# dart-icra/DART-Dual-Arm-Non-Prehensile-Manipulation

Hardware: AMD Instinct MI355X
Metric: MPC solves/sec (horizon N=20, batch=18 objects) at 1/2/4/8 GPUs; max |u−u_ref| (higher is better)
Workload: dtype f64

## Files before the change

dart-dual-arm-non-prehensile-manipulation_amd/csrc/dart_mpc_abi.hip:

```cpp
#include "abi_internal.h"

hipError_t device_stage(DeviceStage** out) {
    static DeviceStage stages[64];
    int dev = 0;
    hipError_t e = hipGetDevice(&dev);
    if (e != hipSuccess) return e;
    if (dev < 0 || dev >= 64) return hipErrorInvalidDevice;
    DeviceStage& d = stages[dev];
    std::lock_guard<std::mutex> g(d.mu);
    if (!d.stream) e = hipStreamCreateWithFlags(&d.stream, hipStreamNonBlocking);
    *out = &d;
    return e;
}

namespace {

int check_cfg(const dart_mpc_config* c) {
    if (!c) return 0;
    if (c->variant != DART_MPC_PMPC && c->variant != DART_MPC_RMPC && c->variant != DART_MPC_LMPC) return 0;
    if (c->N < 1 || c->N > 63) return 0;
    if (!(c->Ts > 0.0) || !(c->tol > 0.0) || !(c->gravity == c->gravity) || c->max_iter < 1 || c->B_max < 1) return 0;
    if (c->acceptable_iter < 0 || (c->acceptable_iter > 0 && !(c->acceptable_tol > 0.0))) return 0;
    if (c->max_soc < 0 || c->max_soc > 8) return 0;
    if (c->pmpc_path != 0 && c->pmpc_path != 1) return 0;
    if (!(c->constr_mult_init_max >= 0.0)) return 0;
    if (!(c->max_cpu_time >= 0.0) || c->max_cpu_time > 1e9) return 0;
    return 1;
}

void server_release(dart_mpc_handle* h) {
    auto& v = h->srv;
    if (v.mbox) (void)hipHostFree(v.mbox);
    if (v.stream) (void)hipStreamDestroy(v.stream);
    v = dart_mpc_handle::Server{};
}

void io_release(dart_mpc_handle* h) {
    auto& o = h->io;
    if (o.hin) (void)hipHostFree(o.hin);
    if (o.hout) (void)hipHostFree(o.hout);
    o = dart_mpc_handle::Io{};
}

hipError_t ensure_io(dart_mpc_handle* h) {
// ... 863 lines not shown
```

dart-dual-arm-non-prehensile-manipulation_amd/csrc/pmpc_ipm.hip:

```cpp
#if DART_WG == 2
#define dartmpc dartmpc_wg2
#endif
#include <hip/hip_runtime.h>
#include <stdint.h>
#include <stdlib.h>

#include "pmpc_ipm.h"
#include "pmpc_model.h"
#include "pmpc_resto.h"
#include "stamps.h"
#include "wave.h"

namespace dartmpc {

#ifdef DART_STAMPS
#ifndef PMPC_SEQ
__device__ unsigned long long g_stamp[16];
#define STAMP_FLUSH(b) STAMP_FLUSH_TO(g_stamp, b)
#else
__device__ unsigned long long g_stamp_seq[16];
#define STAMP_FLUSH(b) STAMP_FLUSH_TO(g_stamp_seq, b)
#endif
#else
#define STAMP_FLUSH(b) STAMP_FLUSH_TO(g_stamp, b)
#endif

#if DART_WG == 2
__shared__ double g_pm_x[4][2][4];
#endif
template <int SITE, int NV>
__device__ __forceinline__ void pm_pass(int src_wave, int src_node, const double (&v)[NV], double (&o)[NV]) {
    static_assert(NV <= 4 && SITE < 4, "four slots, four sites");
#if DART_WG == 1
    (void)src_wave; (void)src_node;
#pragma unroll
    for (int i = 0; i < NV; ++i) o[i] = v[i];
#else
    const int l = lane_id();
    if (wave_idx() == src_wave && (l & 31) == src_node) {
#pragma unroll
        for (int i = 0; i < NV; ++i) g_pm_x[SITE][l >> 5][i] = v[i];
    }
    __syncthreads();
#pragma unroll
// ... 55 lines not shown
    double F[16];
#pragma unroll
    for (int e = 0; e < 16; ++e)
        F[e] = fz[e] ? (e == 0 ? 1.0 : 0.0)
                     : (e % 5 == 0) ? dpp_fill<CTRL, 0xf, 1>(T[e]) : dpp_fill<CTRL, 0xf, 0>(T[e]);
    double N[16];
#pragma unroll
    for (int i = 0; i < 4; ++i)
#pragma unroll
        for (int j = 0; j < 4; ++j) {
            double acc = T[4 * i + 3] * F[12 + j];
            if (fz[12 + j]) acc = 0.0;
            acc = fma(T[4 * i + 2], F[8 + j], acc);
            if (!fz[4 + j]) acc = fma(T[4 * i + 1], F[4 + j], acc);
            if (FIRST && i == 0) acc += F[j];
            else if (!(FIRST && (i == 1 || i == 3))) acc = fma(T[4 * i], F[j], acc);
            N[4 * i + j] = acc;
        }
#pragma unroll
    for (int e = 0; e < 16; ++e) T[e] = N[e];
}

#define PM_EXPECT(x, v) (ONEROW ? (bool)(x) : (bool)__builtin_expect((long)(bool)(x), (v)))

struct PmStage {
    double f11, a12k, a22k, ai12k, ai22k, a22i, uonf, A11k, A12k, A22k;
};

template <int NAX, bool QSCAN, bool ONEROW, bool SHORT2>
__device__ __forceinline__ bool pmpc_riccati(const int lane, const int N, const bool uon, const bool lsm,
                                             const double delta, const double qp2, const double qv2,
                                             const PmStage& c, const double (&be1)[NAX], const double (&be2)[NAX],
                                             const double (&E11)[NAX], const double (&E12)[NAX],
                                             const double (&E22)[NAX], const double (&Rt0)[NAX], double (&P11)[NAX],
                                             double (&P12)[NAX], double (&P22)[NAX], double (&W1)[NAX],
                                             double (&W2)[NAX], double (&iQs)[NAX], bool& use_scan) {
    constexpr bool one_row = ONEROW;
    constexpr bool short2 = SHORT2 && !ONEROW;
    const double f11 = c.f11, a12k = c.a12k, a22k = c.a22k, ai12k = c.ai12k, ai22k = c.ai22k, a22i = c.a22i;
    const double uonf = c.uonf, A11k = c.A11k, A12k = c.A12k, A22k = c.A22k;
    (void)lane; (void)ai12k; (void)ai22k; (void)a22i; (void)uonf;
    const double X11d = lsm ? 1.0 : qp2 + delta, X22d = lsm ? 1.0 : qv2 + delta;
    double Quu[NAX], Rt[NAX];
#pragma unroll
    for (int j = 0; j < NAX; ++j) {
        P11[j] = X11d; P12[j] = 0.0; P22[j] = X22d;
// ... 122 lines not shown
        for (int j = 0; j < NAX; ++j) {
            const double e1 = be1[j], e2 = be2[j];
            const double Q = fma(E11[j], n11[j], fma(E12[j], n12[j], fma(E22[j], n22[j], Rt[j])));
            const double PB1 = fma(n11[j], e1, n12[j] * e2), PB2 = fma(n12[j], e1, n22[j] * e2);
            const double U1 = PB1, U2 = fma(PB1, a12k, PB2 * a22k);
            const double X12 = fma(n11[j], a12k, n12[j] * a22k);
            const double X22 = fma(A11k, n11[j], fma(A12k, n12[j], fma(A22k, n22[j], X22d)));
            const double iQ = frcp(Q);
            const double w1 = iQ * U1, w2 = iQ * U2;
            P11[j] = fma(-w1, U1, fma(f11, n11[j], X11d));
            P12[j] = fma(-w1, U2, X12);
            P22[j] = fma(-w2, U2, X22);
            W1[j] = w1; W2[j] = w2;
            Quu[j] = Q; iQs[j] = iQ;
        }
    }
    bool bad = false;
#pragma unroll
    for (int j = 0; j < NAX; ++j) bad = bad || !(Quu[j] > 0.0) || !isfinite(Quu[j]);
    return !wany(bad);
}

struct PmOvlShared {
    double pt[6][kWave];
    double fc[6][kWave];
    int flag[4];
};
__shared__ PmOvlShared g_pm_ovl;

template <int NAX, bool QSCAN, bool ONEROW, bool SHORT2, bool RED, bool OVL = false>
__device__ __forceinline__ bool pmpc_solve(const PmpcArgs& a, const int b) {
    static_assert(!OVL || (NAX == 1 && QSCAN && !ONEROW && !RED && kWaves == 1), "the overlapped build: scan builds of N = 16..31");
    STAMP_DECL
    const int lane = (kWaves == 1 && !OVL) ? (int)threadIdx.x : lane_id();
    const int k = NAX == 1 ? node_base() + (lane & 31) : lane;
    const int ax0 = NAX == 1 ? (lane >> 5) : 0;
    const int N = a.N;
    const bool xon = k <= N, uon = k < N;
    constexpr bool one_row = ONEROW;
    constexpr bool short2 = SHORT2 && !ONEROW;
    const double h = a.Ts;

    const double* st = a.x0 + 6 * b;
    const double* rf = a.ref + 6 * b;
    const double* pr = a.prm + 6 * b;
    const double mu_f = pr[0], Qp = pr[1], Qv = pr[2], R = pr[3], ulo = pr[4], uhi = pr[5];

    double a12, a22, b1, b2;
    axis_rk4(h, a.g, mu_f, 0.0, 0.0, 1.0, a12, a22);
// ... 26 lines not shown
        v[j] = xon ? (ww ? ww[6 * k + 2 * ax + 1] : sv[j]) : 0.0;
        double t = uon ? (ww ? ww[6 * (N + 1) + 2 * k + ax] : 0.0) : 0.0;
        if (uon) t = fmin(fmax(t, lo + pushl), hi - pushu);
        th[j] = t;
        lp[j] = 0.0; lv[j] = 0.0;
        zl[j] = uon ? 1.0 : 0.0; zu[j] = uon ? 1.0 : 0.0;
        if (xon) gmax = fmax(gmax, fmax(fabs(2 * Qp * (p[j] - rp[j])), fabs(2 * Qv * (v[j] - rv[j]))));
        if (uon) gmax = fmax(gmax, fabs(2 * R * th[j]));
        zA[j] = ax ? zav : zp1; zC[j] = ax ? zcv : zcp;
        zs[j] = st[4 + ax];
        zz[j] = xon ? (ww ? ww[6 * k + 4 + ax] : zs[j]) : 0.0;
    }
    gmax = wmax(gmax);
    const double sc = gmax > 100.0 ? 100.0 / gmax : 1.0;
    const double qp2 = sc * 2 * Qp, qv2 = sc * 2 * Qv, r2 = sc * 2 * R;
    const double scQp = sc * Qp, scQv = sc * Qv, scR = sc * R;
    const PmStage stg = {f11, a12k, a22k, ai12k, ai22k, a22i, uonf, A11k, A12k, A22k};
    auto quad_stage = [&](double csj, double snj, double lpnj, double lvnj, double zlj, double islj, double zuj,
                          double isuj, double& e1, double& e2, double& e11, double& e12, double& e22, double& rt0) {
        e1 = b1 * csj; e2 = b2 * csj;
        e11 = e1 * e1; e12 = 2.0 * e1 * e2; e22 = e2 * e2;
        rt0 = uon ? fma(snj, fma(b1, lpnj, b2 * lvnj), r2 + zlj * islj + zuj * isuj) : 1.0;
    };
    if constexpr (OVL) {
        if (__builtin_amdgcn_readfirstlane((int)(threadIdx.x >> 6)) != 0) {
            const long long max_rounds = 2ll * a.max_iter + 8;
            for (long long round = 0; round < max_rounds; ++round) {
                __syncthreads();
                if (__builtin_amdgcn_readfirstlane(g_pm_ovl.flag[0])) return false;
#ifdef DART_STAMPS
                const unsigned long long tf0 = __builtin_amdgcn_s_memtime();
#endif
                const double th1 = g_pm_ovl.pt[0][lane], sn1 = g_pm_ovl.pt[1][lane];
                const double lp1 = g_pm_ovl.pt[2][lane], lv1 = g_pm_ovl.pt[3][lane];
                const double zl1 = g_pm_ovl.pt[4][lane], zu1 = g_pm_ovl.pt[5][lane];
                const double c_ = tilt_cos_econ(poly, th1);
                const double cs1 = uon ? c_ : 0.0;
                const double ln = from_next(lp1), vn = from_next(lv1);
                const double lpn1 = uon ? ln : 0.0, lvn1 = uon ? vn : 0.0;
                const double sl = th1 - lo, su = hi - th1;
                const double isl1 = uon ? frcp(sl) : 0.0, isu1 = uon ? frcp(su) : 0.0;
                double be1[NAX], be2[NAX], E11[NAX], E12[NAX], E22[NAX], Rt0[NAX];
                quad_stage(cs1, sn1, lpn1, lvn1, zl1, isl1, zu1, isu1, be1[0], be2[0], E11[0], E12[0], E22[0], Rt0[0]);
                double W1[NAX], W2[NAX], P11[NAX], P12[NAX], P22[NAX], iQs[NAX];
                bool us = false;
                const bool okf = pmpc_riccati<NAX, QSCAN, ONEROW, SHORT2>(lane, N, uon, false, 0.0, qp2, qv2, stg, be1,
                                                                         be2, E11, E12, E22, Rt0, P11, P12, P22, W1,
                                                                         W2, iQs, us);
                g_pm_ovl.fc[0][lane] = P11[0]; g_pm_ovl.fc[1][lane] = P12[0]; g_pm_ovl.fc[2][lane] = P22[0];
                g_pm_ovl.fc[3][lane] = W1[0]; g_pm_ovl.fc[4][lane] = W2[0]; g_pm_ovl.fc[5][lane] = iQs[0];
                if (lane == 0) { g_pm_ovl.flag[1] = us ? 1 : 0; g_pm_ovl.flag[2] = okf ? 1 : 0; }
#ifdef DART_STAMPS
                t_acc_[13] += __builtin_amdgcn_s_memtime() - tf0;
                if (lane == 0) g_pm_ovl.flag[3] = (int)t_acc_[13];
#endif
                __syncthreads();
                if (__builtin_amdgcn_readfirstlane(g_pm_ovl.flag[0])) return false;
            }
            return false;
        }
        if (lane == 0) g_pm_ovl.flag[0] = 0;
    }

    const double tol = a.tol, mu_min = tol / 10;
    const double n_eq = 6.0 * (N + 1), n_b = 4.0 * N;
    const double inv_neb = 1.0 / (n_eq + n_b), inv_nb = 1.0 / n_b;
    const double gam_th = 1e-5, gam_ph = 1e-8, s_th = 1.1, s_ph = 2.3, eta_ph = 1e-8, gam_al = 0.05;

    auto defects = [&](double pj, double vj, double sj, double spj, double svj, double& g1, double& g2) {
        const double fp = fma(a12, vj, fma(b1, sj, pj));
        const double fv = fma(a22, vj, b2 * sj);
        double ip, iv;
        if constexpr (kWaves == 1) {
            ip = from_prev(fp); iv = from_prev(fv);
        } else {
            const double x2[2] = {fp, fv};
            double o2[2];
            from_prev_n(x2, o2);
            ip = o2[0]; iv = o2[1];
        }
        g1 = (k == 0) ? pj - spj : pj - ip;
        g2 = (k == 0) ? vj - svj : vj - iv;
    };
    auto axes_sum = [&](const double (&q)[NAX]) -> double {
        if constexpr (NAX == 1) return half_pair_sum(q[0]);
        else return q[0] + q[1];
    };
    auto zdefect = [&](double zj, double wj, int j) -> double {
        const double fz = fma(zA[j], zj, zC[j] * wj);
        const double ip = from_prev(fz);
        return (k == 0) ? zj - zs[j] : zj - ip;
    };
    auto vz_new = [&](const double (&t)[NAX]) -> double {
        double sq[NAX];
#pragma unroll
        for (int j = 0; j < NAX; ++j) sq[j] = uon ? t[j] * t[j] : 0.0;
        return -a.g * axes_sum(sq);
    };

    double g1[NAX], g2[NAX], gz[NAX], snc[NAX];
    double lgc[NAX];
    (void)lgc;
    double th0 = 0.0;
    {
        const double w0 = vz_new(th);
#pragma unroll
        for (int j = 0; j < NAX; ++j) {
            double s0, c0_;
            tilt_sincos(poly, th[j], s0, c0_);
            snc[j] = uon ? s0 : 0.0;
            if constexpr (OVL) lgc[j] = log_fast((th[j] - lo) * (hi - th[j]));
            defects(p[j], v[j], snc[j], sp[j], sv[j], g1[j], g2[j]);
            gz[j] = RED ? 0.0 : zdefect(zz[j], w0, j);
            if (xon) th0 += fabs(g1[j]) + fabs(g2[j]) + fabs(gz[j]);
        }
    }
    double theta = wsum(th0);
    const double th_max = 1e4 * fmax(1.0, theta), th_min = 1e-4 * fmax(1.0, theta);

    double fth = 0.0, fph = 0.0;
    int nfilt = 0;
    double mu = 0.1, delta_last = 0.0;
    int status = -1, it = 0;
    int in_soft = 0, soft_count = 0;
    STAMP(0);

    double zsm[4] = {0.0, 0.0, 0.0, 0.0};
    (void)zsm;
    if constexpr (OVL) {
        double m = k == 0 ? 0.0 : zA[0], c = 0.0;
        affine1_scan_level<0x111, 0xf>(m, c); zsm[0] = m;
        affine1_scan_level<0x112, 0xf>(m, c); zsm[1] = m;
        affine1_scan_level<0x114, 0xf>(m, c); zsm[2] = m;
        if constexpr (!short2) { affine1_scan_level<0x118, 0xf>(m, c); zsm[3] = m; }
    }

    bool published = false;
    auto publish = [&]() {
        __builtin_amdgcn_sched_barrier(0);
        g_pm_ovl.pt[0][lane] = th[0]; g_pm_ovl.pt[1][lane] = snc[0];
        g_pm_ovl.pt[2][lane] = lp[0]; g_pm_ovl.pt[3][lane] = lv[0];
        g_pm_ovl.pt[4][lane] = zl[0]; g_pm_ovl.pt[5][lane] = zu[0];
        __syncthreads();
        __builtin_amdgcn_sched_barrier(0);
        published = true;
    };
#ifdef DART_STAMPS
    const unsigned long long t_loop0 = __builtin_amdgcn_s_memtime();
#endif
    for (it = a.mult_init_max > 0.0 ? -1 : 0; it < a.max_iter; ++it) {
        const bool lsm = it < 0;
#ifdef DART_STAMPS
        if (it == 1) t_acc_[12] = __builtin_amdgcn_s_memtime() - t_loop0;
#endif
        if constexpr (OVL) {
            if (PM_EXPECT(!lsm && !published, 0)) publish();
        }
        double sn[NAX], cs[NAX], isl[NAX], isu[NAX], lpn[NAX], lvn[NAX];
        double dinf = 0.0, pinf = 0.0, c0 = 0.0, cmin = 1e300, suml = 0.0, sumz = 0.0;
#pragma unroll
        for (int j = 0; j < NAX; ++j) {
            sn[j] = snc[j];
            const double c_ = tilt_cos_econ(poly, th[j]);
            cs[j] = uon ? c_ : 0.0;
            double ln, vn;
            if constexpr (kWaves == 1) {
                ln = from_next(lp[j]); vn = from_next(lv[j]);
            } else {
                const double x2[2] = {lp[j], lv[j]};
                double o2[2];
                from_next_n(x2, o2);
                ln = o2[0]; vn = o2[1];
            }
            lpn[j] = uon ? ln : 0.0; lvn[j] = uon ? vn : 0.0;
            const double sl = th[j] - lo, su = hi - th[j];
            isl[j] = uon ? frcp(sl) : 0.0; isu[j] = uon ? frcp(su) : 0.0;
            const double r1 = fma(qp2, p[j] - rp[j], lp[j] - lpn[j]);
            const double r2x = fma(qv2, v[j] - rv[j], lv[j] - fma(a12, lpn[j], a22 * lvn[j]));
            const double ru = fma(r2, th[j], -cs[j] * fma(b1, lpn[j], b2 * lvn[j])) - zl[j] + zu[j];
            dinf = fmax(dinf, xon ? fmax(fabs(r1), fabs(r2x)) : 0.0);
            dinf = fmax(dinf, uon ? fabs(ru) : 0.0);
            pinf = fmax(pinf, xon ? fmax(fmax(fabs(g1[j]), fabs(g2[j])), fabs(gz[j])) : 0.0);
            suml += xon ? fabs(lp[j]) + fabs(lv[j]) : 0.0;
            c0 = fmax(c0, uon ? fmax(zl[j] * sl, zu[j] * su) : 0.0);
            cmin = fmin(cmin, uon ? fmin(zl[j] * sl, zu[j] * su) : 1e300);
            sumz += zl[j] + zu[j];
        }
        float dinf_f = (float)dinf, pinf_f = (float)pinf, c0_f = (float)c0, cmin_f = (float)cmin;
        float suml_f = (float)suml, sumz_f = (float)sumz;
        wred_errors(dinf_f, pinf_f, c0_f, cmin_f, suml_f, sumz_f);
        const double dinf_w = dinf_f, pinf_w = pinf_f, c0_w = c0_f;
        const double cmin_w = cmin_f;
        const float sz_w = sumz_f;
        const double is_d = 100.0 * frcp(fmax(100.0, (double)(suml_f + sz_w) * inv_neb));
        const double is_c = 100.0 * frcp(fmax(100.0, (double)sz_w * inv_nb));
        dinf = dinf_w; pinf = pinf_w; c0 = c0_w;
        STAMP(1);
        if (!lsm && fmax(dinf * is_d, fmax(pinf, c0 * is_c)) <= tol) { status = 0; break; }
        for (; !lsm;) {
            const double cmu = fmax(c0 - mu, mu - cmin_w);
            if (fmax(dinf * is_d, fmax(pinf, cmu * is_c)) > 10.0 * mu || mu <= mu_min) break;
            mu = fmax(mu_min, fmin(0.2 * mu, mu * sqrt(mu)));
            nfilt = 0; in_soft = 0;
        }
        const double tau = fmax(0.99, 1.0 - mu);
        STAMP(2);

        double be1[NAX], be2[NAX], E11[NAX], E12[NAX], E22[NAX], Rt0[NAX], rt[NAX], q1[NAX], q2[NAX];
#pragma unroll
        for (int j = 0; j < NAX; ++j) {
            quad_stage(cs[j], sn[j], lpn[j], lvn[j], zl[j], isl[j], zu[j], isu[j], be1[j], be2[j], E11[j], E12[j],
                       E22[j], Rt0[j]);
            rt[j] = uon ? (lsm ? r2 * th[j] - zl[j] + zu[j] : fma(r2, th[j], mu * (isu[j] - isl[j]))) : 0.0;
            q1[j] = qp2 * (p[j] - rp[j]); q2[j] = qv2 * (v[j] - rv[j]);
        }
        double W1[NAX], W2[NAX], P11[NAX], P12[NAX], P22[NAX], iQs[NAX];
        double delta = 0.0;
        bool ok = false;
        int attempt = 0;
        if constexpr (OVL) {
            if (!lsm) {
                __builtin_amdgcn_sched_barrier(0);
                SPAN_BEGIN(t_b);
                __syncthreads();
                SPAN_END(14, t_b);
                const int usf = g_pm_ovl.flag[1], okff = g_pm_ovl.flag[2];
                P11[0] = g_pm_ovl.fc[0][lane]; P12[0] = g_pm_ovl.fc[1][lane]; P22[0] = g_pm_ovl.fc[2][lane];
                W1[0] = g_pm_ovl.fc[3][lane]; W2[0] = g_pm_ovl.fc[4][lane]; iQs[0] = g_pm_ovl.fc[5][lane];
                const bool us = __builtin_amdgcn_readfirstlane(usf) != 0;
                const bool okf = __builtin_amdgcn_readfirstlane(okff) != 0;
                if (PM_EXPECT(us && okf, 1)) {
                    STAMP_ADD(11, 1);
                    ok = true; attempt = 1;
                }
            }
        }
        for (; attempt < 60 && !ok; ++attempt) {
            if (PM_EXPECT(attempt > 0, 0))
                delta = (attempt == 1) ? (delta_last == 0.0 ? 1e-4 : fmax(1e-20, delta_last * (1.0 / 3.0)))
                                       : delta * (delta_last == 0.0 ? 100.0 : 8.0);
            bool use_scan = false;
            ok = pmpc_riccati<NAX, QSCAN, ONEROW, SHORT2>(lane, N, uon, lsm, delta, qp2, qv2, stg, be1, be2, E11, E12,
                                                          E22, Rt0, P11, P12, P22, W1, W2, iQs, use_scan);
            STAMP_ADD(11, use_scan ? 1 : 0);
        }
        STAMP_ADD(9, attempt);
        STAMP(3);
        if (PM_EXPECT(!ok, 0)) { status = -3; break; }
        if (delta > 0.0) delta_last = delta;

        double dp[NAX], dv[NAX], dth[NAX], dlp[NAX], dlv[NAX], dzl[NAX], dzu[NAX], dz[NAX];
        double amax = 1.0, az = 1.0;
        float am_lf = 1.0f, az_lf = 1.0f;
// ... 345 lines not shown
                wsum2_maxf_min2f(phil, gtdl, tn_w, am_lf, az_lf);
                frac_set();
                phi = phil; gTd = gtdl;
                const float lg_th = theta > 0.0 ? lg2(theta) : -3.0e38f;
                const float lg_gd = gTd < 0.0 ? lg2(-gTd) : 3.0e38f;
                lg_sw = (float)s_th * lg_th - (float)s_ph * lg_gd;
                amin = gam_th;
                if (gTd < 0.0) amin = fmin(gam_th, fmin(gam_ph * theta * frcp(-gTd), (double)__builtin_amdgcn_exp2f(fmaxf(lg_sw, -126.0f))));
                amin *= gam_al;
                tiny = tn_w < 2.2e-15f;
                alpha = amax; amain = amax;
                if constexpr (OVL) {
                    const double thc = fma(alpha, dth[0], th[0]);
                    double s_, c_;
                    tilt_sincos(poly, thc, s_, c_);
                    sn_pre = uon ? s_ : 0.0; sn_pre_on = true;
                    const double il = frcp(thc - lo), iu = frcp(hi - thc);
                    const double zln = fmax(fmin(fma(az, dzl[0], zl[0]), 1e10 * mu * il), 1e-10 * mu * il);
                    const double zun = fmax(fmin(fma(az, dzu[0], zu[0]), 1e10 * mu * iu), 1e-10 * mu * iu);
                    __builtin_amdgcn_sched_barrier(0);
                    g_pm_ovl.pt[0][lane] = thc; g_pm_ovl.pt[1][lane] = sn_pre;
                    g_pm_ovl.pt[2][lane] = fma(alpha, dlp[0], lp[0]); g_pm_ovl.pt[3][lane] = fma(alpha, dlv[0], lv[0]);
                    g_pm_ovl.pt[4][lane] = uon ? zln : 0.0; g_pm_ovl.pt[5][lane] = uon ? zun : 0.0;
                    __syncthreads();
                    __builtin_amdgcn_sched_barrier(0);
                }
            } else if (soc > 0) {
                alpha = amax;
            }
            STAMP(5);
            bool again = false;
            if constexpr ((NAX == 2 || kWaves == 2) && !RED) {
                if (PM_EXPECT(in_soft, 0)) break;
                if (PM_EXPECT(soc < 0 && alpha < amin, 0)) break;
            }
            for (;;) {
                trial(alpha);
                bool ft = false;
                if (PM_EXPECT(soc == 0 && tiny, 0)) { accepted = true; ftype = true; break; }
                if (acceptable(soc > 0 ? amain : alpha, ft)) { accepted = true; ftype = ft; break; }
                if (PM_EXPECT(!RED && soc == 0 && ls == 0 && a.max_soc > 0 && !(th_t < theta), 0)) {
#pragma unroll
                    for (int j = 0; j < NAX; ++j) {
                        g1[j] = fma(alpha, g1[j], g1t[j]); g2[j] = fma(alpha, g2[j], g2t[j]);
                        gz[j] = fma(alpha, gz[j], gzt[j]);
                    }
// ... 104 lines not shown
        if constexpr (OVL) {
            STAMP_ADD(15, hit ? (1ull << 16) : (1ull << 32));
            if (PM_EXPECT(!hit, 0)) {
                __builtin_amdgcn_sched_barrier(0);
                __syncthreads();
                __builtin_amdgcn_sched_barrier(0);
            }
        }
#pragma unroll
        for (int j = 0; j < NAX; ++j) {
            snc[j] = snt[j];
            lp[j] = fma(alpha, dlp[j], lp[j]); lv[j] = fma(alpha, dlv[j], lv[j]);
            th[j] = fma(alpha, dth[j], th[j]);
            if (OVL && PM_EXPECT(hit, 1)) {
                zl[j] = g_pm_ovl.pt[4][lane]; zu[j] = g_pm_ovl.pt[5][lane];
            } else {
                const double il = frcp(th[j] - lo), iu = frcp(hi - th[j]);
                const double zln = fmax(fmin(fma(az, dzl[j], zl[j]), 1e10 * mu * il), 1e-10 * mu * il);
                const double zun = fmax(fmin(fma(az, dzu[j], zu[j]), 1e10 * mu * iu), 1e-10 * mu * iu);
                zl[j] = uon ? zln : 0.0; zu[j] = uon ? zun : 0.0;
            }
        }
        if constexpr (OVL) {
            if (PM_EXPECT(!hit, 0)) publish();
        }
#pragma unroll
        for (int j = 0; j < NAX; ++j) {
            g1[j] = g1t[j]; g2[j] = g2t[j]; gz[j] = gzt[j];
            if constexpr (OVL) lgc[j] = lgt[j];
            p[j] = fma(alpha, dp[j], p[j]); v[j] = fma(alpha, dv[j], v[j]);
            zz[j] = fma(alpha, dz[j], zz[j]);
        }
        theta = th_t;
        STAMP(7);
    }
    if constexpr (OVL) {
        if (lane == 0) g_pm_ovl.flag[0] = 1;
        __syncthreads();
#ifdef DART_STAMPS
        t_acc_[13] = (unsigned)__builtin_amdgcn_readfirstlane(g_pm_ovl.flag[3]);
#endif
    }

    if (PM_EXPECT(status == kPmNeedResto, 0)) {
        if constexpr (NAX == 1 && kWaves == 1 && !RED) {
            if (a.resto_buf) {
                double* ho = a.resto_buf + (size_t)kPmHo * b;
                double* row = ho + kPmHoRow * k;
                if (xon) {
                    row[2 * ax0] = p[0]; row[2 * ax0 + 1] = v[0]; row[4 + ax0] = zz[0];
                    row[8 + 2 * ax0] = lp[0]; row[8 + 2 * ax0 + 1] = lv[0]; row[8 + 4 + ax0] = 0.0;
                }
                if (uon) { row[6 + ax0] = th[0]; row[14 + ax0] = zl[0]; row[16 + ax0] = zu[0]; }
                if (lane < nfilt) { ho[kPmHoFilt + 2 * lane] = fth; ho[kPmHoFilt + 2 * lane + 1] = fph; }
                if (lane == 0) {
                    ho[kPmHoScal] = mu; ho[kPmHoScal + 1] = delta_last;
                    ho[kPmHoScal + 2] = (double)it; ho[kPmHoScal + 3] = (double)nfilt;
                }
            }
        }
        if (lane == 0 && wave_idx() == 0) a.status[b] = status;
        if (a.done && a.resto == 2) {
            __threadfence_system();
// ... 47 lines not shown
    }
    if (a.done) {
        __threadfence_system();
        if constexpr (kWaves == 2) __syncthreads();
        if (lane == 0 && wave_idx() == 0) __hip_atomic_store(a.done + b, a.seq, __ATOMIC_RELAXED, __HIP_MEMORY_SCOPE_SYSTEM);
    }
    STAMP(8);
    STAMP_FLUSH(b);
    return false;
}

__device__ __noinline__ void pmpc_resto_tail(const int b, const uint32_t seq, const uint32_t fl,
                                             const unsigned long long kargs) {
    PmpcArgs a = kernarg_load<PmpcArgs>(kargs);
    a.seq = seq;
    if (!(fl & 1u)) a.w_warm = nullptr;
    if (!(fl & 2u)) a.w_out = nullptr;
    __syncthreads();
    pmpc_resto_solve(a, b);
}

template <int NAX, bool QSCAN, bool ONEROW = false, bool SHORT2 = false, bool RED = false, bool OCC2 = false,
          bool FUSE = false, bool OVL = false>
__global__ __launch_bounds__(kWave * kWaves * (OVL ? 2 : 1)) __attribute__((amdgpu_waves_per_eu(OCC2 ? 2 : ((QSCAN || NAX == 2) ? 1 : 2))))
void pmpc_ipm_kernel(PmpcArgs a) {
    if (blockIdx.x % a.pack) return;
    const int b = blockIdx.x / a.pack;
    const bool handed = pmpc_solve<NAX, QSCAN, ONEROW, SHORT2, RED, OVL>(a, b);
    if constexpr (FUSE) {
        if (PM_EXPECT(handed, 0)) pmpc_resto_tail(b, a.seq, 3u, kernarg_addr());
    }
}

template <int NAX, bool ONEROW, bool SHORT2, bool FUSE = false>
__global__ __launch_bounds__(kWave) __attribute__((amdgpu_waves_per_eu(1)))
void pmpc_serve_kernel(PmpcArgs a, PmpcServe sv) {
    if (blockIdx.x % a.pack) return;
    const int b = blockIdx.x / a.pack;
    uint32_t seen = a.seq;
    unsigned long long t_last = __builtin_amdgcn_s_memrealtime();
    for (;;) {
        const unsigned long long w =
            __hip_atomic_load((const unsigned long long*)sv.mailbox, __ATOMIC_ACQUIRE, __HIP_MEMORY_SCOPE_SYSTEM);
        const uint32_t lo = (uint32_t)__builtin_amdgcn_readfirstlane((int)(uint32_t)(w & 0xffffffffu));
        const uint32_t hi = (uint32_t)__builtin_amdgcn_readfirstlane((int)(uint32_t)(w >> 32));
        const uint32_t sq = lo;
        if (hi >> 24) break;
// ... 63 lines not shown
                           stream, *a);
    else
        hipLaunchKernelGGL((dartmpc::pmpc_ipm_kernel<2, false, false, false, RED>), dim3(grid), dim3(dartmpc::kWave), 0,
                           stream, *a);
}
extern "C" hipError_t dartmpc_launch_pmpc_seq(const dartmpc::PmpcArgs* a, unsigned grid, hipStream_t stream,
                                              int onerow) {
    if (a->reduced) launch_seq<true>(a, grid, stream, onerow);
    else launch_seq<false>(a, grid, stream, onerow);
    return hipGetLastError();
}
extern "C" hipError_t dartmpc_launch_pmpc_serve_onerow(const dartmpc::PmpcArgs* a, const dartmpc::PmpcServe* sv,
                                                      unsigned grid, hipStream_t stream) {
    if (a->resto == 3)
        hipLaunchKernelGGL((dartmpc::pmpc_serve_kernel<1, true, false, true>), dim3(grid), dim3(dartmpc::kWave), 0,
                           stream, *a, *sv);
    else
        hipLaunchKernelGGL((dartmpc::pmpc_serve_kernel<1, true, false>), dim3(grid), dim3(dartmpc::kWave), 0, stream,
                           *a, *sv);
    return hipGetLastError();
}
#ifdef DART_STAMPS
extern "C" hipError_t dartmpc_read_stamps_seq(unsigned long long* host_out) {
    return hipMemcpyFromSymbol(host_out, HIP_SYMBOL(dartmpc::g_stamp_seq), sizeof(unsigned long long) * 16, 0,
                               hipMemcpyDeviceToHost);
}
#endif
#else
extern "C" hipError_t dartmpc_launch_pmpc_seq(const dartmpc::PmpcArgs* a, unsigned grid, hipStream_t stream,
                                              int onerow);
extern "C" hipError_t dartmpc_launch_pmpc_serve_onerow(const dartmpc::PmpcArgs* a, const dartmpc::PmpcServe* sv,
                                                      unsigned grid, hipStream_t stream);
extern "C" hipError_t dartmpc_launch_pmpc_wg2(const void* args, unsigned grid, hipStream_t stream);

extern "C" hipError_t dartmpc_launch_pmpc_serve(const dartmpc::PmpcArgs* args, const dartmpc::PmpcServe* sv,
                                               hipStream_t stream) {
    if (args->B <= 0 || args->N > 31) return hipErrorInvalidValue;
    dartmpc::PmpcArgs a = *args;
    a.pack = (a.B <= 32) ? 8 : 1;
    if (a.resto && a.pack == 8 && dartmpc::resto_fuse_enabled()) a.resto = 3;
    else if (a.resto) a.resto = 2;
    const unsigned grid = (unsigned)(a.B * a.pack);
    if (a.N <= 15) return dartmpc_launch_pmpc_serve_onerow(&a, sv, grid, stream);
    if (a.N <= 23 && a.resto == 3)
        hipLaunchKernelGGL((dartmpc::pmpc_serve_kernel<1, false, true, true>), dim3(grid), dim3(dartmpc::kWave), 0,
                           stream, a, *sv);
    else if (a.N <= 23)
// ... 15 lines not shown
    const dim3 grid(a.B * a.pack);
    static const int qscan_max_b = [] {
        const char* e = getenv("DART_PMPC_QSCAN_MAX_B");
        return e ? atoi(e) : (1 << 30);
    }();
    static const int occ2_min_b = [] {
        if (const char* e = getenv("DART_PMPC_OCC2_MIN_B")) return atoi(e);
        int dev = 0, cus = 0;
        if (hipGetDevice(&dev) != hipSuccess || hipDeviceGetAttribute(&cus, hipDeviceAttributeMultiprocessorCount, dev) != hipSuccess || cus <= 0)
            return 1 << 30;
        return 2 * 4 * cus;
    }();
    const bool occ2 = !a.reduced && a.B >= occ2_min_b && a.B <= qscan_max_b;
    static const bool long_wg2 = [] {
        const char* e = getenv("DART_PMPC_SEQ_LONG");
        return !(e && e[0] == '1');
    }();
    if (a.resto == 1 && a.pack == 8 && !a.reduced && a.N <= 31 && !occ2 && a.B <= qscan_max_b &&
        dartmpc::resto_fuse_enabled())
        a.resto = 3;
    const bool fuse = a.resto == 3;
    const bool ovl = a.pack == 8 && !a.reduced && !occ2 && a.N >= 16 && a.N <= 31 && a.B <= qscan_max_b &&
                     dartmpc::pmpc_overlap_enabled();
    const dim3 block2(2 * dartmpc::kWave);
    if (ovl && a.N <= 23) {
        if (fuse)
            hipLaunchKernelGGL((dartmpc::pmpc_ipm_kernel<1, true, false, true, false, false, true, true>), grid, block2, 0, stream, a);
        else
            hipLaunchKernelGGL((dartmpc::pmpc_ipm_kernel<1, true, false, true, false, false, false, true>), grid, block2, 0, stream, a);
    } else if (ovl) {
        if (fuse)
            hipLaunchKernelGGL((dartmpc::pmpc_ipm_kernel<1, true, false, false, false, false, true, true>), grid, block2, 0, stream, a);
        else
            hipLaunchKernelGGL((dartmpc::pmpc_ipm_kernel<1, true, false, false, false, false, false, true>), grid, block2, 0, stream, a);
    } else if (a.N <= 23 && occ2) {
        hipLaunchKernelGGL((dartmpc::pmpc_ipm_kernel<1, true, false, true, false, true>), grid, dim3(dartmpc::kWave), 0, stream, a);
    } else if (a.N <= 15 && a.B <= qscan_max_b) {
        if (hipError_t e = dartmpc_launch_pmpc_seq(&a, grid.x, stream, 1)) return e;
    } else if (a.N <= 23 && a.B <= qscan_max_b) {
        if (fuse)
            hipLaunchKernelGGL((dartmpc::pmpc_ipm_kernel<1, true, false, true, false, false, true>), grid, dim3(dartmpc::kWave), 0, stream, a);
        else if (a.reduced)
            hipLaunchKernelGGL((dartmpc::pmpc_ipm_kernel<1, true, false, true, true>), grid, dim3(dartmpc::kWave), 0, stream, a);
        else
            hipLaunchKernelGGL((dartmpc::pmpc_ipm_kernel<1, true, false, true>), grid, dim3(dartmpc::kWave), 0, stream, a);
    } else if (a.N <= 31 && a.B <= qscan_max_b) {
        if (occ2)
            hipLaunchKernelGGL((dartmpc::pmpc_ipm_kernel<1, true, false, false, false, true>), grid, dim3(dartmpc::kWave), 0, stream, a);
        else if (fuse)
            hipLaunchKernelGGL((dartmpc::pmpc_ipm_kernel<1, true, false, false, false, false, true>), grid, dim3(dartmpc::kWave), 0, stream, a);
        else if (a.reduced)
            hipLaunchKernelGGL((dartmpc::pmpc_ipm_kernel<1, true, false, false, true>), grid, dim3(dartmpc::kWave), 0, stream, a);
        else
            hipLaunchKernelGGL((dartmpc::pmpc_ipm_kernel<1, true>), grid, dim3(dartmpc::kWave), 0, stream, a);
    } else if (a.N > 31 && !a.reduced && !a.resto && long_wg2) {
        if (hipError_t e = dartmpc_launch_pmpc_wg2(&a, grid.x, stream)) return e;
    } else {
        if (hipError_t e = dartmpc_launch_pmpc_seq(&a, grid.x, stream, 0)) return e;
    }
    if (a.resto == 1) {
        if (hipError_t e = hipGetLastError()) return e;
        return dartmpc_launch_pmpc_resto(&a, stream);
    }
    return hipGetLastError();
}

extern "C" hipError_t dartmpc_wave_selftest(double* d_out, hipStream_t stream) {
    hipLaunchKernelGGL(dartmpc::wave_selftest_kernel, dim3(1), dim3(dartmpc::kWave), 0, stream, d_out);
    return hipGetLastError();
}

#ifdef DART_STAMPS
extern "C" hipError_t dartmpc_read_stamps(unsigned long long* host_out) {
    return hipMemcpyFromSymbol(host_out, HIP_SYMBOL(dartmpc::g_stamp), sizeof(unsigned long long) * 16, 0,
                               hipMemcpyDeviceToHost);
}
#endif
#endif
```

Baseline: 337,700.

## Offload IPM convergence check and mu update to a third helper wave

Adds a third wave to the overlapped PMPC kernel. It evaluates the KKT residuals, convergence verdict and barrier-parameter update on the published trial point while the main wave runs its step. The main wave skips its own error reductions and mu loop, and instead reads the verdict, the new mu and the filter-reset flag from shared memory after the barrier. This takes the reduction-heavy termination check off the critical path. The cost is a larger block, more shared-memory traffic, and a one-round lag structure whose correctness depends on the helper seeing the accepted point.

```diff
diff --git a/dart-dual-arm-non-prehensile-manipulation_amd/csrc/dart_mpc_abi.hip b/dart-dual-arm-non-prehensile-manipulation_amd/csrc/dart_mpc_abi.hip
--- a/dart-dual-arm-non-prehensile-manipulation_amd/csrc/dart_mpc_abi.hip
+++ b/dart-dual-arm-non-prehensile-manipulation_amd/csrc/dart_mpc_abi.hip
@@ -19,7 +19,8 @@
     if (!c) return 0;
     if (c->variant != DART_MPC_PMPC && c->variant != DART_MPC_RMPC && c->variant != DART_MPC_LMPC) return 0;
     if (c->N < 1 || c->N > 63) return 0;
-    if (!(c->Ts > 0.0) || !(c->tol > 0.0) || !(c->gravity == c->gravity) || c->max_iter < 1 || c->B_max < 1) return 0;
+    if (!(c->Ts > 0.0) || !(c->tol > 0.0) || !(c->gravity == c->gravity) || c->B_max < 1) return 0;
+    if (c->max_iter < (c->variant == DART_MPC_PMPC ? 0 : 1)) return 0;
     if (c->acceptable_iter < 0 || (c->acceptable_iter > 0 && !(c->acceptable_tol > 0.0))) return 0;
     if (c->max_soc < 0 || c->max_soc > 8) return 0;
     if (c->pmpc_path != 0 && c->pmpc_path != 1) return 0;
diff --git a/dart-dual-arm-non-prehensile-manipulation_amd/csrc/pmpc_ipm.hip b/dart-dual-arm-non-prehensile-manipulation_amd/csrc/pmpc_ipm.hip
--- a/dart-dual-arm-non-prehensile-manipulation_amd/csrc/pmpc_ipm.hip
+++ b/dart-dual-arm-non-prehensile-manipulation_amd/csrc/pmpc_ipm.hip
@@ -15,11 +15,11 @@
 
 #ifdef DART_STAMPS
 #ifndef PMPC_SEQ
-__device__ unsigned long long g_stamp[16];
-#define STAMP_FLUSH(b) STAMP_FLUSH_TO(g_stamp, b)
+__device__ unsigned long long g_stamp[32];
+#define STAMP_FLUSH(b) STAMP_FLUSH32_TO(g_stamp, b)
 #else
-__device__ unsigned long long g_stamp_seq[16];
-#define STAMP_FLUSH(b) STAMP_FLUSH_TO(g_stamp_seq, b)
+__device__ unsigned long long g_stamp_seq[32];
+#define STAMP_FLUSH(b) STAMP_FLUSH32_TO(g_stamp_seq, b)
 #endif
 #else
 #define STAMP_FLUSH(b) STAMP_FLUSH_TO(g_stamp, b)
@@ -121,6 +121,13 @@
 }
 
 #define PM_EXPECT(x, v) (ONEROW ? (bool)(x) : (bool)__builtin_expect((long)(bool)(x), (v)))
+
+__device__ __forceinline__ double wave_uniform(double x) {
+    const unsigned long long b = __builtin_bit_cast(unsigned long long, x);
+    const unsigned lo = (unsigned)__builtin_amdgcn_readfirstlane((int)(unsigned)(b & 0xffffffffu));
+    const unsigned hi = (unsigned)__builtin_amdgcn_readfirstlane((int)(unsigned)(b >> 32));
+    return __builtin_bit_cast(double, ((unsigned long long)hi << 32) | lo);
+}
 
 struct PmStage {
     double f11, a12k, a22k, ai12k, ai22k, a22i, uonf, A11k, A12k, A22k;
@@ -289,9 +296,10 @@
 }
 
 struct PmOvlShared {
-    double pt[6][kWave];
+    double pt[10][kWave];
     double fc[6][kWave];
-    int flag[4];
+    double mu_new;
+    int flag[8];
 };
 __shared__ PmOvlShared g_pm_ovl;
 
@@ -364,12 +372,99 @@
         e11 = e1 * e1; e12 = 2.0 * e1 * e2; e22 = e2 * e2;
         rt0 = uon ? fma(snj, fma(b1, lpnj, b2 * lvnj), r2 + zlj * islj + zuj * isuj) : 1.0;
     };
+    const double tol = a.tol, mu_min = tol / 10;
+    const double n_eq = 6.0 * (N + 1), n_b = 4.0 * N;
+    const double inv_neb = 1.0 / (n_eq + n_b), inv_nb = 1.0 / n_b;
+    const double gam_th = 1e-5, gam_ph = 1e-8, s_th = 1.1, s_ph = 2.3, eta_ph = 1e-8, gam_al = 0.05;
+
+    auto defects = [&](double pj, double vj, double sj, double spj, double svj, double& g1, double& g2) {
+        const double fp = fma(a12, vj, fma(b1, sj, pj));
+        const double fv = fma(a22, vj, b2 * sj);
+        double ip, iv;
+        if constexpr (kWaves == 1) {
+            ip = from_prev(fp); iv = from_prev(fv);
+        } else {
+            const double x2[2] = {fp, fv};
+            double o2[2];
+            from_prev_n(x2, o2);
+            ip = o2[0]; iv = o2[1];
+        }
+        g1 = (k == 0) ? pj - spj : pj - ip;
+        g2 = (k == 0) ? vj - svj : vj - iv;
+    };
+    auto axes_sum = [&](const double (&q)[NAX]) -> double {
+        if constexpr (NAX == 1) return half_pair_sum(q[0]);
+        else return q[0] + q[1];
+    };
+    auto zdefect = [&](double zj, double wj, int j) -> double {
+        const double fz = fma(zA[j], zj, zC[j] * wj);
+        const double ip = from_prev(fz);
+        return (k == 0) ? zj - zs[j] : zj - ip;
+    };
+    auto vz_new = [&](const double (&t)[NAX]) -> double {
+        double sq[NAX];
+#pragma unroll
+        for (int j = 0; j < NAX; ++j) sq[j] = uon ? t[j] * t[j] : 0.0;
+        return -a.g * axes_sum(sq);
+    };
+
+    auto point_verdict = [&](const double (&p)[NAX], const double (&v)[NAX], const double (&th)[NAX],
+                             const double (&lp)[NAX], const double (&lv)[NAX], const double (&zl)[NAX],
+                             const double (&zu)[NAX], const double (&g1)[NAX], const double (&g2)[NAX],
+                             const double (&gz)[NAX], double& mu, bool& dec) -> bool {
+        double dinf = 0.0, pinf = 0.0, c0 = 0.0, cmin = 1e300, suml = 0.0, sumz = 0.0;
+#pragma unroll
+        for (int j = 0; j < NAX; ++j) {
+            const double c_ = tilt_cos_econ(poly, th[j]);
+            const double cs = uon ? c_ : 0.0;
+            const double ln = from_next(lp[j]), vn = from_next(lv[j]);
+            const double lpn = uon ? ln : 0.0, lvn = uon ? vn : 0.0;
+            const double sl = th[j] - lo, su = hi - th[j];
+            const double r1 = fma(qp2, p[j] - rp[j], lp[j] - lpn);
+            const double r2x = fma(qv2, v[j] - rv[j], lv[j] - fma(a12, lpn, a22 * lvn));
+            const double ru = fma(r2, th[j], -cs * fma(b1, lpn, b2 * lvn)) - zl[j] + zu[j];
+            dinf = fmax(dinf, xon ? fmax(fabs(r1), fabs(r2x)) : 0.0);
+            dinf = fmax(dinf, uon ? fabs(ru) : 0.0);
+            pinf = fmax(pinf, xon ? fmax(fmax(fabs(g1[j]), fabs(g2[j])), fabs(gz[j])) : 0.0);
+            suml += xon ? fabs(lp[j]) + fabs(lv[j]) : 0.0;
+            c0 = fmax(c0, uon ? fmax(zl[j] * sl, zu[j] * su) : 0.0);
+            cmin = fmin(cmin, uon ? fmin(zl[j] * sl, zu[j] * su) : 1e300);
+            sumz += zl[j] + zu[j];
+        }
+        float dinf_f = (float)dinf, pinf_f = (float)pinf, c0_f = (float)c0, cmin_f = (float)cmin;
+        float suml_f = (float)suml, sumz_f = (float)sumz;
+        wred_errors(dinf_f, pinf_f, c0_f, cmin_f, suml_f, sumz_f);
+        const double dinf_w = dinf_f, pinf_w = pinf_f, c0_w = c0_f;
+        const double cmin_w = cmin_f;
+        const float sz_w = sumz_f;
+        const double is_d = 100.0 * frcp(fmax(100.0, (double)(suml_f + sz_w) * inv_neb));
+        const double is_c = 100.0 * frcp(fmax(100.0, (double)sz_w * inv_nb));
+        dinf = dinf_w; pinf = pinf_w; c0 = c0_w;
+        dec = false;
+        if (fmax(dinf * is_d, fmax(pinf, c0 * is_c)) <= tol) return true;
+        for (;;) {
+            const double cmu = fmax(c0 - mu, mu - cmin_w);
+            if (fmax(dinf * is_d, fmax(pinf, cmu * is_c)) > 10.0 * mu || mu <= mu_min) break;
+            mu = fmax(mu_min, fmin(0.2 * mu, mu * sqrt(mu)));
+            dec = true;
+        }
+        return false;
+    };
+    (void)point_verdict;
     if constexpr (OVL) {
-        if (__builtin_amdgcn_readfirstlane((int)(threadIdx.x >> 6)) != 0) {
+        auto helper_rounds = [&](auto&& body) {
             const long long max_rounds = 2ll * a.max_iter + 8;
             for (long long round = 0; round < max_rounds; ++round) {
                 __syncthreads();
-                if (__builtin_amdgcn_readfirstlane(g_pm_ovl.flag[0])) return false;
+                if (__builtin_amdgcn_readfirstlane(g_pm_ovl.flag[0])) return;
+                body();
+                __syncthreads();
+                if (__builtin_amdgcn_readfirstlane(g_pm_ovl.flag[0])) return;
+            }
+        };
+        const int wv = __builtin_amdgcn_readfirstlane((int)(threadIdx.x >> 6));
+        if (wv == 1) {
+            helper_rounds([&]() {
 #ifdef DART_STAMPS
                 const unsigned long long tf0 = __builtin_amdgcn_s_memtime();
 #endif
@@ -396,49 +491,36 @@
                 t_acc_[13] += __builtin_amdgcn_s_memtime() - tf0;
                 if (lane == 0) g_pm_ovl.flag[3] = (int)t_acc_[13];
 #endif
-                __syncthreads();
-                if (__builtin_amdgcn_readfirstlane(g_pm_ovl.flag[0])) return false;
-            }
+            });
             return false;
         }
+        if (wv == 2) {
+            helper_rounds([&]() {
+#ifdef DART_STAMPS
+                const unsigned long long te0 = __builtin_amdgcn_s_memtime();
+#endif
+                const double th1[NAX] = {g_pm_ovl.pt[0][lane]}, sn1 = g_pm_ovl.pt[1][lane];
+                const double lp1[NAX] = {g_pm_ovl.pt[2][lane]}, lv1[NAX] = {g_pm_ovl.pt[3][lane]};
+                const double zl1[NAX] = {g_pm_ovl.pt[4][lane]}, zu1[NAX] = {g_pm_ovl.pt[5][lane]};
+                const double p1[NAX] = {g_pm_ovl.pt[6][lane]}, v1[NAX] = {g_pm_ovl.pt[7][lane]};
+                const double zz1 = g_pm_ovl.pt[8][lane];
+                double mu1 = wave_uniform(g_pm_ovl.pt[9][lane]);
+                double g1e[NAX], g2e[NAX], gze[NAX];
+                const double w1 = vz_new(th1);
+                defects(p1[0], v1[0], sn1, sp[0], sv[0], g1e[0], g2e[0]);
+                gze[0] = zdefect(zz1, w1, 0);
+                bool dec = false;
+                const bool conv = point_verdict(p1, v1, th1, lp1, lv1, zl1, zu1, g1e, g2e, gze, mu1, dec);
+                if (lane == 0) { g_pm_ovl.mu_new = mu1; g_pm_ovl.flag[4] = conv ? 1 : 0; g_pm_ovl.flag[5] = dec ? 1 : 0; }
+#ifdef DART_STAMPS
+                t_acc_[17] += __builtin_amdgcn_s_memtime() - te0;
+                if (lane == 0) g_pm_ovl.flag[6] = (int)t_acc_[17];
+#endif
+            });
+            return false;
+        }
         if (lane == 0) g_pm_ovl.flag[0] = 0;
     }
-
-    const double tol = a.tol, mu_min = tol / 10;
-    const double n_eq = 6.0 * (N + 1), n_b = 4.0 * N;
-    const double inv_neb = 1.0 / (n_eq + n_b), inv_nb = 1.0 / n_b;
-    const double gam_th = 1e-5, gam_ph = 1e-8, s_th = 1.1, s_ph = 2.3, eta_ph = 1e-8, gam_al = 0.05;
-
-    auto defects = [&](double pj, double vj, double sj, double spj, double svj, double& g1, double& g2) {
-        const double fp = fma(a12, vj, fma(b1, sj, pj));
-        const double fv = fma(a22, vj, b2 * sj);
-        double ip, iv;
-        if constexpr (kWaves == 1) {
-            ip = from_prev(fp); iv = from_prev(fv);
-        } else {
-            const double x2[2] = {fp, fv};
-            double o2[2];
-            from_prev_n(x2, o2);
-            ip = o2[0]; iv = o2[1];
-        }
-        g1 = (k == 0) ? pj - spj : pj - ip;
-        g2 = (k == 0) ? vj - svj : vj - iv;
-    };
-    auto axes_sum = [&](const double (&q)[NAX]) -> double {
-        if constexpr (NAX == 1) return half_pair_sum(q[0]);
-        else return q[0] + q[1];
-    };
-    auto zdefect = [&](double zj, double wj, int j) -> double {
-        const double fz = fma(zA[j], zj, zC[j] * wj);
-        const double ip = from_prev(fz);
-        return (k == 0) ? zj - zs[j] : zj - ip;
-    };
-    auto vz_new = [&](const double (&t)[NAX]) -> double {
-        double sq[NAX];
-#pragma unroll
-        for (int j = 0; j < NAX; ++j) sq[j] = uon ? t[j] * t[j] : 0.0;
-        return -a.g * axes_sum(sq);
-    };
 
     double g1[NAX], g2[NAX], gz[NAX], snc[NAX];
     double lgc[NAX];
@@ -483,6 +565,8 @@
         g_pm_ovl.pt[0][lane] = th[0]; g_pm_ovl.pt[1][lane] = snc[0];
         g_pm_ovl.pt[2][lane] = lp[0]; g_pm_ovl.pt[3][lane] = lv[0];
         g_pm_ovl.pt[4][lane] = zl[0]; g_pm_ovl.pt[5][lane] = zu[0];
+        g_pm_ovl.pt[6][lane] = p[0]; g_pm_ovl.pt[7][lane] = v[0];
+        g_pm_ovl.pt[8][lane] = zz[0]; g_pm_ovl.pt[9][lane] = mu;
         __syncthreads();
         __builtin_amdgcn_sched_barrier(0);
         published = true;
@@ -517,9 +601,11 @@
             lpn[j] = uon ? ln : 0.0; lvn[j] = uon ? vn : 0.0;
             const double sl = th[j] - lo, su = hi - th[j];
             isl[j] = uon ? frcp(sl) : 0.0; isu[j] = uon ? frcp(su) : 0.0;
+            STAMP(16);
             const double r1 = fma(qp2, p[j] - rp[j], lp[j] - lpn[j]);
             const double r2x = fma(qv2, v[j] - rv[j], lv[j] - fma(a12, lpn[j], a22 * lvn[j]));
             const double ru = fma(r2, th[j], -cs[j] * fma(b1, lpn[j], b2 * lvn[j])) - zl[j] + zu[j];
+            if constexpr (!OVL) {
             dinf = fmax(dinf, xon ? fmax(fabs(r1), fabs(r2x)) : 0.0);
             dinf = fmax(dinf, uon ? fabs(ru) : 0.0);
             pinf = fmax(pinf, xon ? fmax(fmax(fabs(g1[j]), fabs(g2[j])), fabs(gz[j])) : 0.0);
@@ -527,10 +613,11 @@
             c0 = fmax(c0, uon ? fmax(zl[j] * sl, zu[j] * su) : 0.0);
             cmin = fmin(cmin, uon ? fmin(zl[j] * sl, zu[j] * su) : 1e300);
             sumz += zl[j] + zu[j];
+            }
         }
         float dinf_f = (float)dinf, pinf_f = (float)pinf, c0_f = (float)c0, cmin_f = (float)cmin;
         float suml_f = (float)suml, sumz_f = (float)sumz;
-        wred_errors(dinf_f, pinf_f, c0_f, cmin_f, suml_f, sumz_f);
+        if constexpr (!OVL) wred_errors(dinf_f, pinf_f, c0_f, cmin_f, suml_f, sumz_f);
         const double dinf_w = dinf_f, pinf_w = pinf_f, c0_w = c0_f;
         const double cmin_w = cmin_f;
         const float sz_w = sumz_f;
@@ -538,14 +625,18 @@
         const double is_c = 100.0 * frcp(fmax(100.0, (double)sz_w * inv_nb));
         dinf = dinf_w; pinf = pinf_w; c0 = c0_w;
         STAMP(1);
+        if constexpr (!OVL) {
         if (!lsm && fmax(dinf * is_d, fmax(pinf, c0 * is_c)) <= tol) { status = 0; break; }
+        }
+        if constexpr (!OVL) {
         for (; !lsm;) {
             const double cmu = fmax(c0 - mu, mu - cmin_w);
             if (fmax(dinf * is_d, fmax(pinf, cmu * is_c)) > 10.0 * mu || mu <= mu_min) break;
             mu = fmax(mu_min, fmin(0.2 * mu, mu * sqrt(mu)));
             nfilt = 0; in_soft = 0;
         }
-        const double tau = fmax(0.99, 1.0 - mu);
+        }
+        double tau = fmax(0.99, 1.0 - mu);
         STAMP(2);
 
         double be1[NAX], be2[NAX], E11[NAX], E12[NAX], E22[NAX], Rt0[NAX], rt[NAX], q1[NAX], q2[NAX];
@@ -553,7 +644,7 @@
         for (int j = 0; j < NAX; ++j) {
             quad_stage(cs[j], sn[j], lpn[j], lvn[j], zl[j], isl[j], zu[j], isu[j], be1[j], be2[j], E11[j], E12[j],
                        E22[j], Rt0[j]);
-            rt[j] = uon ? (lsm ? r2 * th[j] - zl[j] + zu[j] : fma(r2, th[j], mu * (isu[j] - isl[j]))) : 0.0;
+            if (!OVL || lsm) rt[j] = uon ? (lsm ? r2 * th[j] - zl[j] + zu[j] : fma(r2, th[j], mu * (isu[j] - isl[j]))) : 0.0;
             q1[j] = qp2 * (p[j] - rp[j]); q2[j] = qv2 * (v[j] - rv[j]);
         }
         double W1[NAX], W2[NAX], P11[NAX], P12[NAX], P22[NAX], iQs[NAX];
@@ -567,10 +658,17 @@
                 __syncthreads();
                 SPAN_END(14, t_b);
                 const int usf = g_pm_ovl.flag[1], okff = g_pm_ovl.flag[2];
+                const int cvf = g_pm_ovl.flag[4], mdf = g_pm_ovl.flag[5];
+                const double mun = g_pm_ovl.mu_new;
                 P11[0] = g_pm_ovl.fc[0][lane]; P12[0] = g_pm_ovl.fc[1][lane]; P22[0] = g_pm_ovl.fc[2][lane];
                 W1[0] = g_pm_ovl.fc[3][lane]; W2[0] = g_pm_ovl.fc[4][lane]; iQs[0] = g_pm_ovl.fc[5][lane];
                 const bool us = __builtin_amdgcn_readfirstlane(usf) != 0;
                 const bool okf = __builtin_amdgcn_readfirstlane(okff) != 0;
+                if (__builtin_amdgcn_readfirstlane(cvf)) { status = 0; break; }
+                mu = wave_uniform(mun);
+                if (__builtin_amdgcn_readfirstlane(mdf)) { nfilt = 0; in_soft = 0; }
+                tau = fmax(0.99, 1.0 - mu);
+                rt[0] = uon ? fma(r2, th[0], mu * (isu[0] - isl[0])) : 0.0;
                 if (PM_EXPECT(us && okf, 1)) {
                     STAMP_ADD(11, 1);
                     ok = true; attempt = 1;
@@ -962,6 +1060,8 @@
                     g_pm_ovl.pt[0][lane] = thc; g_pm_ovl.pt[1][lane] = sn_pre;
                     g_pm_ovl.pt[2][lane] = fma(alpha, dlp[0], lp[0]); g_pm_ovl.pt[3][lane] = fma(alpha, dlv[0], lv[0]);
                     g_pm_ovl.pt[4][lane] = uon ? zln : 0.0; g_pm_ovl.pt[5][lane] = uon ? zun : 0.0;
+                    g_pm_ovl.pt[6][lane] = fma(alpha, dp[0], p[0]); g_pm_ovl.pt[7][lane] = fma(alpha, dv[0], v[0]);
+                    g_pm_ovl.pt[8][lane] = fma(alpha, dz[0], zz[0]); g_pm_ovl.pt[9][lane] = mu;
                     __syncthreads();
                     __builtin_amdgcn_sched_barrier(0);
                 }
@@ -1112,14 +1212,18 @@
             }
         }
         if constexpr (OVL) {
+            p[0] = fma(alpha, dp[0], p[0]); v[0] = fma(alpha, dv[0], v[0]);
+            zz[0] = fma(alpha, dz[0], zz[0]);
             if (PM_EXPECT(!hit, 0)) publish();
         }
 #pragma unroll
         for (int j = 0; j < NAX; ++j) {
             g1[j] = g1t[j]; g2[j] = g2t[j]; gz[j] = gzt[j];
             if constexpr (OVL) lgc[j] = lgt[j];
-            p[j] = fma(alpha, dp[j], p[j]); v[j] = fma(alpha, dv[j], v[j]);
-            zz[j] = fma(alpha, dz[j], zz[j]);
+            if constexpr (!OVL) {
+                p[j] = fma(alpha, dp[j], p[j]); v[j] = fma(alpha, dv[j], v[j]);
+                zz[j] = fma(alpha, dz[j], zz[j]);
+            }
         }
         theta = th_t;
         STAMP(7);
@@ -1129,6 +1233,7 @@
         __syncthreads();
 #ifdef DART_STAMPS
         t_acc_[13] = (unsigned)__builtin_amdgcn_readfirstlane(g_pm_ovl.flag[3]);
+        t_acc_[17] = (unsigned)__builtin_amdgcn_readfirstlane(g_pm_ovl.flag[6]);
 #endif
     }
 
@@ -1222,7 +1327,7 @@
 
 template <int NAX, bool QSCAN, bool ONEROW = false, bool SHORT2 = false, bool RED = false, bool OCC2 = false,
           bool FUSE = false, bool OVL = false>
-__global__ __launch_bounds__(kWave * kWaves * (OVL ? 2 : 1)) __attribute__((amdgpu_waves_per_eu(OCC2 ? 2 : ((QSCAN || NAX == 2) ? 1 : 2))))
+__global__ __launch_bounds__(kWave * kWaves * (OVL ? 3 : 1)) __attribute__((amdgpu_waves_per_eu(OCC2 ? 2 : ((QSCAN || NAX == 2) ? 1 : 2))))
 void pmpc_ipm_kernel(PmpcArgs a) {
     if (blockIdx.x % a.pack) return;
     const int b = blockIdx.x / a.pack;
@@ -1332,7 +1437,7 @@
 }
 #ifdef DART_STAMPS
 extern "C" hipError_t dartmpc_read_stamps_seq(unsigned long long* host_out) {
-    return hipMemcpyFromSymbol(host_out, HIP_SYMBOL(dartmpc::g_stamp_seq), sizeof(unsigned long long) * 16, 0,
+    return hipMemcpyFromSymbol(host_out, HIP_SYMBOL(dartmpc::g_stamp_seq), sizeof(unsigned long long) * 32, 0,
                                hipMemcpyDeviceToHost);
 }
 #endif
@@ -1394,17 +1499,17 @@
     const bool fuse = a.resto == 3;
     const bool ovl = a.pack == 8 && !a.reduced && !occ2 && a.N >= 16 && a.N <= 31 && a.B <= qscan_max_b &&
                      dartmpc::pmpc_overlap_enabled();
-    const dim3 block2(2 * dartmpc::kWave);
+    const dim3 block3(3 * dartmpc::kWave);
     if (ovl && a.N <= 23) {
         if (fuse)
-            hipLaunchKernelGGL((dartmpc::pmpc_ipm_kernel<1, true, false, true, false, false, true, true>), grid, block2, 0, stream, a);
+            hipLaunchKernelGGL((dartmpc::pmpc_ipm_kernel<1, true, false, true, false, false, true, true>), grid, block3, 0, stream, a);
         else
-            hipLaunchKernelGGL((dartmpc::pmpc_ipm_kernel<1, true, false, true, false, false, false, true>), grid, block2, 0, stream, a);
+            hipLaunchKernelGGL((dartmpc::pmpc_ipm_kernel<1, true, false, true, false, false, false, true>), grid, block3, 0, stream, a);
     } else if (ovl) {
         if (fuse)
-            hipLaunchKernelGGL((dartmpc::pmpc_ipm_kernel<1, true, false, false, false, false, true, true>), grid, block2, 0, stream, a);
+            hipLaunchKernelGGL((dartmpc::pmpc_ipm_kernel<1, true, false, false, false, false, true, true>), grid, block3, 0, stream, a);
         else
-            hipLaunchKernelGGL((dartmpc::pmpc_ipm_kernel<1, true, false, false, false, false, false, true>), grid, block2, 0, stream, a);
+            hipLaunchKernelGGL((dartmpc::pmpc_ipm_kernel<1, true, false, false, false, false, false, true>), grid, block3, 0, stream, a);
     } else if (a.N <= 23 && occ2) {
         hipLaunchKernelGGL((dartmpc::pmpc_ipm_kernel<1, true, false, true, false, true>), grid, dim3(dartmpc::kWave), 0, stream, a);
     } else if (a.N <= 15 && a.B <= qscan_max_b) {
@@ -1444,7 +1549,7 @@
 
 #ifdef DART_STAMPS
 extern "C" hipError_t dartmpc_read_stamps(unsigned long long* host_out) {
-    return hipMemcpyFromSymbol(host_out, HIP_SYMBOL(dartmpc::g_stamp), sizeof(unsigned long long) * 16, 0,
+    return hipMemcpyFromSymbol(host_out, HIP_SYMBOL(dartmpc::g_stamp), sizeof(unsigned long long) * 32, 0,
                                hipMemcpyDeviceToHost);
 }
 #endif
```

After: 342,000 (median of 6 runs). 1.01x the previous value.
